# choyingw/SynergyNet

Measured on AMD Instinct MI355X. Metric: faces/sec (120x120, 68-lmk + 53215-vert), higher is better.
Workload: dtype f32 (fp16x2 split operands, fp32 accumulate)

## Files before the change

synergynet_amd/csrc/fused_block_lb.hip:

```cpp
#include "syn_internal.h"

#include <cstdio>
#include <cstdlib>

namespace syn {

typedef float f32x4 __attribute__((ext_vector_type(4)));
typedef float f32x2 __attribute__((ext_vector_type(2)));
typedef unsigned u32x4 __attribute__((ext_vector_type(4)));
typedef unsigned u32x2 __attribute__((ext_vector_type(2)));
typedef _Float16 f16x8 __attribute__((ext_vector_type(8)));
typedef _Float16 f16x2 __attribute__((ext_vector_type(2)));

namespace {
__device__ __forceinline__ void split2h(float x0, float x1, unsigned &a, unsigned &b) {
    a = __builtin_bit_cast(unsigned, __builtin_amdgcn_cvt_pkrtz(x0, x1));
    float r0, r1;
    asm("v_fma_mix_f32 %0, %1, -1.0, %2 op_sel_hi:[1,0,0]" : "=v"(r0) : "v"(a), "v"(x0));
    asm("v_fma_mix_f32 %0, %1, -1.0, %2 op_sel:[1,0,0] op_sel_hi:[1,0,0]" : "=v"(r1) : "v"(a), "v"(x1));
    b = __builtin_bit_cast(unsigned, __builtin_amdgcn_cvt_pkrtz(r0, r1));
}
__device__ __forceinline__ void split2v(float x0, float x1, u32x4 (&pc)[2], int d) {
    unsigned a, b;
    split2h(x0, x1, a, b);
// ... 34 lines not shown
__device__ __forceinline__ f32x2 pk_fma_clamp01(f32x2 a, f32x2 b, f32x2 c) {
    f32x2 r;
    asm("v_pk_fma_f32 %0, %1, %2, %3 clamp" : "=v"(r) : "v"(a), "v"(b), "v"(c));
    return r;
}
constexpr int kRowShr1 = 0x111, kRowShl1 = 0x101, kRowShr8 = 0x118, kRowShl8 = 0x108;
constexpr int kRowShr4 = 0x114, kRowShr5 = 0x115;
}

template <int CIN_, int HID_, int COUT_, bool RES_, int EPF_, int PPF_, int FPW_ = 2, bool S2_ = false, int NS_ = 2>
struct LbCfg {
    static constexpr int CIN = CIN_, HID = HID_, COUT = COUT_, FPW = FPW_;
    static constexpr int PPF = PPF_;
    static constexpr bool TLATE = false;
    static constexpr int EPF = EPF_;
    static constexpr bool RES = RES_;
    static constexpr bool S2 = S2_;
    static constexpr int NB = S2 ? 1 : 4;
    static constexpr int PIXO = NB * 16;
    static constexpr int KE = CIN / 32;
    static constexpr int NG = HID / 32;
    static constexpr int MT = COUT / 16;
    static constexpr int NS = NS_;
    static constexpr int NW = FPW * NS, NT = NW * 64;
    static constexpr int XF_DW = KE * 4 * 2 * 256;
    static constexpr int NSX = NS == 8 ? 4 : NS;
    static constexpr int KT = (MT + NSX - 1) / NSX;
    static constexpr int RED_DW = (NS == 2 ? 1 : NSX) * MT * NB * 256;
    static constexpr int TB_DW = 12 * 32;
    static constexpr int FACE_DW = XF_DW > RED_DW ? XF_DW : RED_DW;
    static constexpr int LDS_DW = FPW * FACE_DW + NW * TB_DW;
    static_assert(CIN % 32 == 0 && HID % 64 == 0 && COUT % 32 == 0, "k32 steps, two streams, two halves of the output tiles");
    static_assert(NS == 2 || (NS == 8 && FPW == 1 && (HID / 32) >= NS), "eight streams: the one-face-per-workgroup schedule of small batches (the four-stream form of round 4 is retired)");
    static_assert(EPF == 1 || EPF == KE, "expand prefetch depth");
    static_assert(!RES || (CIN == COUT && !S2), "residual only on same-width stride-1 blocks");
    static_assert((FPW == 4 || NS >= 4 ? 1 : 2) * LDS_DW * 4 <= 160 * 1024, "one 8-wave or two 4-wave workgroups per CU");
};

#define SYNL_FENCE() do { asm volatile("" ::: "memory"); __builtin_amdgcn_sched_barrier(0); } while (0)

#define SYNL_LAP(i) do { if (PROF) { tn = __builtin_amdgcn_s_memtime(); pt_[i] += tn - tk; tk = tn; } } while (0)

struct LbStageArgs {
    const float *X;
    const unsigned *Weh;
    const float *Tlb;
    const unsigned *Wlb;
    const float *p_shift;
    float *Y;
    float *part = nullptr;
    int gsl = 0;
};

template <class C, class CN, bool FIRST, bool PROF, int FACE_DW, bool STORE = true, bool PARTIAL = false, int RED_OFF = 0>
__device__ __forceinline__ void lb_stage(unsigned *smem, const LbStageArgs &sa, int B, unsigned long long (&pt_)[5], unsigned long long &tk) {
    unsigned long long tn = 0;
    const float *__restrict__ X = sa.X;
    const unsigned *__restrict__ Weh = sa.Weh, *__restrict__ Wlb = sa.Wlb;
    const float *__restrict__ Tlb = sa.Tlb, *__restrict__ p_shift = sa.p_shift;
    float *__restrict__ Y = sa.Y;
    constexpr int KE = C::KE, MT = C::MT, CIN = C::CIN, COUT = C::COUT, NB = C::NB;
    const int tid = threadIdx.x, lane = tid & 63;
    const int wave = __builtin_amdgcn_readfirstlane(tid >> 6);
    const int fl = wave / C::NS, st = wave % C::NS;
    const int f = blockIdx.x * C::FPW + fl;
    const bool real = f < B;
    const int fc = real ? f : B - 1;
    const int n = lane & 15, g = lane >> 4;
    const unsigned l4 = lane * 4, g4 = g * 4;
    unsigned *Xf = smem + fl * FACE_DW;
    constexpr int BPW = 4 / C::NS;
    auto pix_in = [&](int b, int nn) __attribute__((always_inline)) {
        return C::S2 ? 16 * (nn >> 2) + 8 * (b >> 1) + 2 * (nn & 3) + (b & 1) : 32 * (nn >> 3) + (nn & 7) + 8 * b;
    };

    if constexpr (FIRST && C::NS == 8) {
        constexpr int NIT = (KE * 4 + 7) / 8;
        f32x4 xv[NIT][2];
#pragma unroll
        for (int i = 0; i < NIT; ++i) {
            const int it = st + 8 * i, itc = it < KE * 4 ? it : 0;
            const float *src = X + ((size_t)fc * 64 + pix_in(itc & 3, n)) * CIN + 32 * (itc >> 2) + 8 * g;
            xv[i][0] = *(const f32x4 *)src;
            xv[i][1] = *(const f32x4 *)(src + 4);
        }
#pragma unroll
        for (int i = 0; i < NIT; ++i) {
            const int it = st + 8 * i;
            f32x4 a = xv[i][0], b = xv[i][1];
            if (!real) { a = (f32x4){0.f, 0.f, 0.f, 0.f}; b = a; }
            a *= 16.0f; b *= 16.0f;
            u32x4 pc[2];
            split2v(a[0], a[1], pc, 0);
            split2v(a[2], a[3], pc, 1);
            split2v(b[0], b[1], pc, 2);
            split2v(b[2], b[3], pc, 3);
            if (it < KE * 4) {
#pragma unroll
                for (int p = 0; p < 2; ++p) *(u32x4 *)&Xf[(it * 2 + p) * 256 + lane * 4] = pc[p];
            }
        }
    } else if (FIRST) {
        f32x4 xv[KE][BPW][2];
#pragma unroll
        for (int kc = 0; kc < KE; ++kc)
#pragma unroll
            for (int rr = 0; rr < BPW; ++rr) {
// ... 145 lines not shown
            for (int r = 0; r < NB; ++r) {
                split2v(O[r][0], O[r][1], Bd[r], th);
                if (hf) {
#pragma unroll
                    for (int p = 0; p < 2; ++p) asm volatile("" : "+v"(Bd[r][p]));
                }
            }
            SYNL_FENCE();
        }
        SYNL_LAP(2);
        const bool more = G + C::NS < gend;
#pragma unroll
        for (int i = 1; i < C::PPF; ++i)
            if (i < MT) fetch_p(i);
        if (more) {
            if (!C::TLATE) fetch_t(G + C::NS);
            if (C::EPF != KE) {
#pragma unroll
                for (int kc = 0; kc < C::EPF; ++kc) fetch_e(G + C::NS, kc);
            }
        }
        if constexpr (C::S2) {
            static_assert(!C::S2 || (C::PPF == 2 && MT % 2 == 0), "output tiles in pairs, two tiles fetched ahead");
#pragma unroll
            for (int mt = 0; mt < MT; mt += 2) {
                if (mt + 2 < MT) { fetch_p(mt + 2); fetch_p(mt + 3); }
                constexpr int PA[3] = {1, 0, 0}, PB[3] = {0, 1, 0};
#pragma unroll
                for (int j = 0; j < 3; ++j) {
                    acc[mt][0] = mfmal(Ap[mt % RING][PA[j]], Bd[0][PB[j]], acc[mt][0]);
                    acc[mt + 1][0] = mfmal(Ap[(mt + 1) % RING][PA[j]], Bd[0][PB[j]], acc[mt + 1][0]);
                }
                SYNL_FENCE();
            }
        } else {
#pragma unroll
            for (int mt = 0; mt < MT; ++mt) {
                if (mt + C::PPF < MT) fetch_p(mt + C::PPF);
                mac3x4(Ap[mt % RING], Bd[0], acc[mt][0], Ap[mt % RING], Bd[1], acc[mt][1], Ap[mt % RING], Bd[2], acc[mt][2], Ap[mt % RING], Bd[3], acc[mt][3]);
                SYNL_FENCE();
            }
        }
        if (more) {
            if (C::TLATE) fetch_t(G + C::NS);
            park_t();
        }
        SYNL_LAP(3);
    }

    float *Red = reinterpret_cast<float *>(Xf + RED_OFF);
    int le = lane;
    asm volatile("" : "+v"(le));
    const int ne = le & 15, ge = le >> 4, pixe = C::S2 ? ne : 32 * (ne >> 3) + (ne & 7);
    const __amdgpu_buffer_rsrc_t rs_x = __builtin_amdgcn_make_buffer_rsrc(const_cast<float *>(X), 0, 0x7fffffff, 0x00027000);
    constexpr int KT = C::KT, NSW = C::NSX;
    f32x4 rs[KT][NB], psh[KT];
#pragma unroll
    for (int i = 0; i < KT; ++i) {
        const int mtk = NSW * i + (st & (NSW - 1));
        const int nch = 16 * (mtk < MT ? mtk : MT - 1) + 4 * ge;
        psh[i] = *(const f32x4 *)&p_shift[nch];
#pragma unroll
        for (int r = 0; r < NB; ++r)
            if (C::RES && !PARTIAL) rs[i][r] = __builtin_bit_cast(f32x4, __builtin_amdgcn_raw_buffer_load_b128(rs_x, (unsigned)(((fc * 64 + pixe + 8 * r) * COUT + nch) * 4), 0, FIRST ? 0 : 1));
    }
    if (RED_OFF == 0) __syncthreads();
    constexpr bool HANDOFF = !__is_same(CN, void);
    f32x4 vout[KT][NB];
    if constexpr (C::NS == 2) {
#pragma unroll
    for (int mt = 0; mt < MT; ++mt) {
        if ((mt & 1) == st) continue;
#pragma unroll
        for (int r = 0; r < NB; ++r) *(f32x4 *)&Red[(((st * (MT / 2) + (mt >> 1)) * NB + r) * 64 + lane) * 4] = acc[mt][r];
    }
    __syncthreads();
#pragma unroll
    for (int mt = 0; mt < MT; ++mt) {
        if ((mt & 1) != st) continue;
        const int nch = 16 * mt + 4 * ge;
#pragma unroll
        for (int r = 0; r < NB; ++r) {
            const f32x4 o = *(const f32x4 *)&Red[((((1 - st) * (MT / 2) + (mt >> 1)) * NB + r) * 64 + lane) * 4];
            f32x4 v = st == 0 ? acc[mt][r] + o : o + acc[mt][r];
            if constexpr (PARTIAL) {
                if (real) *(f32x4 *)&sa.part[(((size_t)blockIdx.y * B + f) * C::PIXO + pixe + 8 * r) * COUT + nch] = v;
                continue;
            }
            v = v * inv_p + psh[mt >> 1];
            if (C::RES) v += rs[mt >> 1][r];
            if (STORE && real) *(f32x4 *)&Y[((size_t)f * C::PIXO + pixe + 8 * r) * COUT + nch] = v;
            if (HANDOFF) vout[mt >> 1][r] = v;
        }
    }
    } else {
        static_assert(!PARTIAL, "the four-stream schedule reduces inside the workgroup");
        if constexpr (C::NS == 8) {
            if (st >= 4) {
#pragma unroll
                for (int mt = 0; mt < MT; ++mt)
#pragma unroll
                    for (int r = 0; r < NB; ++r) *(f32x4 *)&Red[((((st - 4) * MT + mt) * NB + r) * 64 + lane) * 4] = acc[mt][r];
            }
            __syncthreads();
            if (st < 4) {
#pragma unroll
                for (int mt = 0; mt < MT; ++mt)
#pragma unroll
                    for (int r = 0; r < NB; ++r) acc[mt][r] += *(const f32x4 *)&Red[(((st * MT + mt) * NB + r) * 64 + lane) * 4];
            }
            __syncthreads();
        }
#pragma unroll
        for (int mt = 0; mt < MT; ++mt) {
            if (mt % NSW == st || st >= NSW) continue;
#pragma unroll
            for (int r = 0; r < NB; ++r) *(f32x4 *)&Red[(((st * MT + mt) * NB + r) * 64 + lane) * 4] = acc[mt][r];
        }
        __syncthreads();
#pragma unroll
        for (int mt = 0; mt < MT; ++mt) {
            if (mt % NSW != st) continue;
            const int nch = 16 * mt + 4 * ge;
#pragma unroll
            for (int r = 0; r < NB; ++r) {
                f32x4 v = st == 0 ? acc[mt][r] : *(const f32x4 *)&Red[(((0 * MT + mt) * NB + r) * 64 + lane) * 4];
#pragma unroll
                for (int so = 1; so < NSW; ++so) v += so == st ? acc[mt][r] : *(const f32x4 *)&Red[(((so * MT + mt) * NB + r) * 64 + lane) * 4];
                v = v * inv_p + psh[mt / NSW];
                if (C::RES) v += rs[mt / NSW][r];
                if (STORE && real) *(f32x4 *)&Y[((size_t)f * C::PIXO + pixe + 8 * r) * COUT + nch] = v;
                if (HANDOFF) vout[mt / NSW][r] = v;
            }
        }
    }
    if constexpr (HANDOFF) {
        static_assert(CN::CIN == COUT && !C::S2, "the next block of the chain takes this block's output (8x8)");
        if (RED_OFF == 0) __syncthreads();
#pragma unroll
        for (int mt = 0; mt < MT; ++mt) {
            if (mt % NSW != st) continue;
            const int kc = mt >> 1, lg = (2 * (mt & 1) + (ge >> 1)) * 16, dw = 2 * (ge & 1);
#pragma unroll
            for (int r = 0; r < 4; ++r) {
                const f32x4 v = real ? vout[mt / NSW][r] * 16.0f : (f32x4){0.f, 0.f, 0.f, 0.f};
                unsigned a0, b0, a1, b1;
                split2h(v[0], v[1], a0, b0);
                split2h(v[2], v[3], a1, b1);
                const int bn = CN::S2 ? 2 * (r & 1) + (ne & 1) : r;
                const int nn = CN::S2 ? 4 * ((r >> 1) + 2 * (ne >> 3)) + ((ne & 7) >> 1) : ne;
                *(u32x2 *)&Xf[((kc * 4 + bn) * 2 + 0) * 256 + (lg + nn) * 4 + dw] = (u32x2){a0, a1};
                *(u32x2 *)&Xf[((kc * 4 + bn) * 2 + 1) * 256 + (lg + nn) * 4 + dw] = (u32x2){b0, b1};
            }
        }
    }
    SYNL_LAP(4);
}

struct L7 {
    static constexpr int CIN = 32, HID = 192, COUT = 64, NG = 6, MT = 4, H = 15, HO = 8;
    static constexpr int FPW = 2, NW = 4, NT = 256;
    static constexpr int XF_DW = 16 * 2 * 256;
    static constexpr int TB_DW = 12 * 32;
    static constexpr int FACE_DW = XF_DW;
    static constexpr int LDS_DW = FPW * FACE_DW + NW * TB_DW;
};

template <class CN, bool PROF, int FACE_DW>
__device__ __forceinline__ void lb7_stage(unsigned *smem, const LbStageArgs &sa, int B, unsigned long long (&pt_)[5], unsigned long long &tk) {
    unsigned long long tn = 0;
    const float *__restrict__ X = sa.X;
    const float *__restrict__ Tlb = sa.Tlb, *__restrict__ p_shift = sa.p_shift;
    float *__restrict__ Y = sa.Y;
    constexpr int MT = L7::MT, CIN = L7::CIN, COUT = L7::COUT;
    const int tid = threadIdx.x, lane = tid & 63;
    const int wave = __builtin_amdgcn_readfirstlane(tid >> 6);
    const int fl = wave >> 1, st = wave & 1;
    const int f = blockIdx.x * L7::FPW + fl;
    const bool real = f < B;
    const int fc = real ? f : B - 1;
    const int n = lane & 15, g = lane >> 4;
    const unsigned l4 = lane * 4, g4 = g * 4;
    unsigned *Xf = smem + fl * FACE_DW;

#pragma unroll
    for (int hb = 0; hb < 2; ++hb) {
        f32x4 xv[4][2];
        bool ok[4];
#pragma unroll
        for (int b = 0; b < 4; ++b) {
            const int y = 2 * (2 * b + (n >> 3)) + st, x = 2 * (n & 7) + hb;
            ok[b] = real && y < L7::H && x < L7::H;
            const float *src = X + ((size_t)fc * (L7::H * L7::H) + (ok[b] ? y * L7::H + x : 0)) * CIN + 8 * g;
            xv[b][0] = *(const f32x4 *)src;
            xv[b][1] = *(const f32x4 *)(src + 4);
        }
#pragma unroll
        for (int b = 0; b < 4; ++b) {
            f32x4 a = xv[b][0], c = xv[b][1];
            if (!ok[b]) { a = (f32x4){0.f, 0.f, 0.f, 0.f}; c = a; }
            a *= 16.0f; c *= 16.0f;
            u32x4 pc[2];
            split2v(a[0], a[1], pc, 0);
            split2v(a[2], a[3], pc, 1);
            split2v(c[0], c[1], pc, 2);
            split2v(c[2], c[3], pc, 3);
#pragma unroll
            for (int p = 0; p < 2; ++p) *(u32x4 *)&Xf[((((2 * st + hb) * 4 + b) * 2) + p) * 256 + lane * 4] = pc[p];
        }
    }
    const float mL = (n & 7) != 0 ? 1.f : 0.f;
    f32x4 acc[MT][2];
#pragma unroll
    for (int mt = 0; mt < MT; ++mt)
#pragma unroll
        for (int k = 0; k < 2; ++k) acc[mt][k] = (f32x4){0.f, 0.f, 0.f, 0.f};

    float *Tb = reinterpret_cast<float *>(smem + L7::FPW * FACE_DW + wave * L7::TB_DW);
    const __amdgpu_buffer_rsrc_t rs_e = __builtin_amdgcn_make_buffer_rsrc(const_cast<unsigned *>(sa.Weh), 0, 0x7fffffff, 0x00027000);
    const __amdgpu_buffer_rsrc_t rs_p = __builtin_amdgcn_make_buffer_rsrc(const_cast<unsigned *>(sa.Wlb), 0, 0x7fffffff, 0x00027000);
    const __amdgpu_buffer_rsrc_t rs_t = __builtin_amdgcn_make_buffer_rsrc(const_cast<float *>(Tlb), 0, 0x7fffffff, 0x00027000);
// ... 78 lines not shown
            };
            f32x2 up2, up3;
            if (st == 1) {
                up2 = dpp2<kRowShl8>(relu(D[t][2][2], c6e));
                up3 = dpp2<kRowShl8>(relu(D[t][3][2], cJ));
            } else {
                up2 = (f32x2){0.f, 0.f}; up3 = up2;
            }
#pragma unroll
            for (int k = 0; k < 2; ++k) {
                const f32x2 E0 = relu(D[t][0][k], c6e), E1 = relu(D[t][1][k], cJ);
                const f32x2 E2 = relu(D[t][2][k], k == 1 ? cR0 : c6e), E3 = relu(D[t][3][k], k == 1 ? cR1 : cJ);
                const f32x2 U2 = dpp2<kRowShr8>(E2) + up2, U3 = dpp2<kRowShr8>(E3) + up3;
                f32x2 O = dsh;
                O += dpp2<kRowShr1>(U3) * w[0];
                O += U2 * w[1];
                O += U3 * w[2];
                asm volatile("" : "+v"(O));
                O += dpp2<kRowShr1>(E1) * w[3];
                O += E0 * w[4];
                O += E1 * w[5];
                asm volatile("" : "+v"(O));
                O += dpp2<kRowShr1>(E3) * w[6];
                O += E2 * w[7];
                O = pk_fma_clamp01(E3, w[8], O);
                split2v(O[0], O[1], Bd[k], th);
                if (k == 0) { up2 = dpp2<kRowShl8>(E2); up3 = dpp2<kRowShl8>(E3); }
            }
            SYNL_FENCE();
        }
        SYNL_LAP(2);
        const bool more = G + 1 < L7::NG;
        fetch_p(1);
        if (more) { fetch_t(G + 1); fetch_e(G + 1); }
#pragma unroll
        for (int mt = 0; mt < MT; ++mt) {
            if (mt + 2 < MT) fetch_p(mt + 2);
            constexpr int PA[3] = {1, 0, 0}, PB[3] = {0, 1, 0};
#pragma unroll
            for (int j = 0; j < 3; ++j) {
                acc[mt][0] = mfmal(Ap[mt % 3][PA[j]], Bd[0][PB[j]], acc[mt][0]);
                acc[mt][1] = mfmal(Ap[mt % 3][PA[j]], Bd[1][PB[j]], acc[mt][1]);
            }
            SYNL_FENCE();
        }
        if (more) park_t();
        SYNL_LAP(3);
    }

    int le = lane;
    asm volatile("" : "+v"(le));
    const int ne = le & 15, ge = le >> 4, ox = ne & 7;
    constexpr bool HANDOFF = !__is_same(CN, void);
    if constexpr (HANDOFF) __syncthreads();
#pragma unroll
    for (int mt = 0; mt < MT; ++mt) {
        const int nch = 16 * mt + 4 * ge;
        const f32x4 psh = *(const f32x4 *)&p_shift[nch];
#pragma unroll
        for (int k = 0; k < 2; ++k) {
            const int oy = 4 * st + 2 * k + (ne >> 3);
            const f32x4 v = acc[mt][k] * inv_p + psh;
            if (real) *(f32x4 *)&Y[((size_t)f * 64 + oy * 8 + ox) * COUT + nch] = v;
            if constexpr (HANDOFF) {
                static_assert(CN::CIN == COUT && !CN::S2, "features.8 takes this block's output");
                const int kc = mt >> 1, lg = (2 * (mt & 1) + (ge >> 1)) * 16, dw = 2 * (ge & 1);
                const int r = 2 * k + (ne >> 3), nn = 8 * st + ox;
                const f32x4 vs = real ? v * 16.0f : (f32x4){0.f, 0.f, 0.f, 0.f};
                unsigned a0, b0, a1, b1;
                split2h(vs[0], vs[1], a0, b0);
                split2h(vs[2], vs[3], a1, b1);
                *(u32x2 *)&Xf[((kc * 4 + r) * 2 + 0) * 256 + (lg + nn) * 4 + dw] = (u32x2){a0, a1};
                *(u32x2 *)&Xf[((kc * 4 + r) * 2 + 1) * 256 + (lg + nn) * 4 + dw] = (u32x2){b0, b1};
            }
        }
    }
    SYNL_LAP(4);
}

template <class CN, int FACE_DW>
__device__ __forceinline__ void lb7_stage8(unsigned *smem, const LbStageArgs &sa, int B) {
    const float *__restrict__ X = sa.X;
    const float *__restrict__ Tlb = sa.Tlb, *__restrict__ p_shift = sa.p_shift;
    float *__restrict__ Y = sa.Y;
    constexpr int MT = L7::MT, CIN = L7::CIN, COUT = L7::COUT;
    const int tid = threadIdx.x, lane = tid & 63;
    const int wave = __builtin_amdgcn_readfirstlane(tid >> 6);
    const int q = wave & 3, hs = wave >> 2;
    const int f = blockIdx.x;
    const bool real = f < B;
    const int fc = real ? f : B - 1;
    const int n = lane & 15, g = lane >> 4;
    const unsigned l4 = lane * 4, g4 = g * 4;
    unsigned *Xf = smem;

    {
        const int c = wave & 3, py = c >> 1, px = c & 1, b0 = 2 * (wave >> 2);
        f32x4 xv[2][2];
        bool ok[2];
#pragma unroll
        for (int bb = 0; bb < 2; ++bb) {
            const int b = b0 + bb;
            const int y = 2 * (2 * b + (n >> 3)) + py, x = 2 * (n & 7) + px;
            ok[bb] = real && y < L7::H && x < L7::H;
            const float *src = X + ((size_t)fc * (L7::H * L7::H) + (ok[bb] ? y * L7::H + x : 0)) * CIN + 8 * g;
            xv[bb][0] = *(const f32x4 *)src;
            xv[bb][1] = *(const f32x4 *)(src + 4);
        }
#pragma unroll
        for (int bb = 0; bb < 2; ++bb) {
            f32x4 a = xv[bb][0], d = xv[bb][1];
            if (!ok[bb]) { a = (f32x4){0.f, 0.f, 0.f, 0.f}; d = a; }
            a *= 16.0f; d *= 16.0f;
            u32x4 pc[2];
            split2v(a[0], a[1], pc, 0);
            split2v(a[2], a[3], pc, 1);
            split2v(d[0], d[1], pc, 2);
            split2v(d[2], d[3], pc, 3);
#pragma unroll
            for (int p = 0; p < 2; ++p) *(u32x4 *)&Xf[(((c * 4 + b0 + bb) * 2) + p) * 256 + lane * 4] = pc[p];
        }
    }
    const float mL = (n & 7) != 0 ? 1.f : 0.f;
    f32x4 acc[MT];
#pragma unroll
    for (int mt = 0; mt < MT; ++mt) acc[mt] = (f32x4){0.f, 0.f, 0.f, 0.f};

    float *Tb = reinterpret_cast<float *>(smem + FACE_DW + wave * L7::TB_DW);
    const __amdgpu_buffer_rsrc_t rs_e = __builtin_amdgcn_make_buffer_rsrc(const_cast<unsigned *>(sa.Weh), 0, 0x7fffffff, 0x00027000);
    const __amdgpu_buffer_rsrc_t rs_p = __builtin_amdgcn_make_buffer_rsrc(const_cast<unsigned *>(sa.Wlb), 0, 0x7fffffff, 0x00027000);
    const __amdgpu_buffer_rsrc_t rs_t = __builtin_amdgcn_make_buffer_rsrc(const_cast<float *>(Tlb), 0, 0x7fffffff, 0x00027000);
    const unsigned l16 = lane * 16;
    f32x4 tv[2];
// ... 76 lines not shown
                up2 = dpp2<kRowShl8>(relu(Dh[t][0], c6e));
                up3 = dpp2<kRowShl8>(relu(Dh[t][1], cJ));
            } else {
                up2 = (f32x2){0.f, 0.f}; up3 = up2;
            }
            const f32x2 E0 = relu(D[t][0], c6e), E1 = relu(D[t][1], cJ);
            const f32x2 E2 = relu(D[t][2], cR0), E3 = relu(D[t][3], cR1);
            const f32x2 U2 = dpp2<kRowShr8>(E2) + up2, U3 = dpp2<kRowShr8>(E3) + up3;
            f32x2 O = dsh;
            O += dpp2<kRowShr1>(U3) * w[0];
            O += U2 * w[1];
            O += U3 * w[2];
            asm volatile("" : "+v"(O));
            O += dpp2<kRowShr1>(E1) * w[3];
            O += E0 * w[4];
            O += E1 * w[5];
            asm volatile("" : "+v"(O));
            O += dpp2<kRowShr1>(E3) * w[6];
            O += E2 * w[7];
            O = pk_fma_clamp01(E3, w[8], O);
            split2v(O[0], O[1], Bd, th);
            SYNL_FENCE();
        }
        const bool more = G + 2 < L7::NG;
        fetch_p(1);
        if (more) { fetch_t(G + 2); fetch_e(G + 2); }
#pragma unroll
        for (int mt = 0; mt < MT; ++mt) {
            if (mt + 2 < MT) fetch_p(mt + 2);
            constexpr int PA[3] = {1, 0, 0}, PB[3] = {0, 1, 0};
#pragma unroll
            for (int j = 0; j < 3; ++j) acc[mt] = mfmal(Ap[mt % 3][PA[j]], Bd[PB[j]], acc[mt]);
            SYNL_FENCE();
        }
        if (more) park_t();
    }

    float *Ex = reinterpret_cast<float *>(Xf);
    int le = lane;
    asm volatile("" : "+v"(le));
    const int ne = le & 15, ge = le >> 4, ox = ne & 7, oy = 2 * q + (ne >> 3);
    __syncthreads();
    if (hs == 1) {
#pragma unroll
        for (int mt = 0; mt < MT; ++mt) *(f32x4 *)&Ex[((q * MT + mt) * 64 + lane) * 4] = acc[mt];
    }
    __syncthreads();
    f32x4 v[MT];
    if (hs == 0) {
#pragma unroll
        for (int mt = 0; mt < MT; ++mt) {
            const int nch = 16 * mt + 4 * ge;
            v[mt] = (acc[mt] + *(const f32x4 *)&Ex[((q * MT + mt) * 64 + lane) * 4]) * inv_p + *(const f32x4 *)&p_shift[nch];
            if (real) *(f32x4 *)&Y[((size_t)f * 64 + oy * 8 + ox) * COUT + nch] = v[mt];
        }
    }
    static_assert(CN::CIN == COUT && !CN::S2, "features.8 takes this block's output");
    __syncthreads();
    if (hs == 0) {
#pragma unroll
        for (int mt = 0; mt < MT; ++mt) {
            const int kc = mt >> 1, lg = (2 * (mt & 1) + (ge >> 1)) * 16, dw = 2 * (ge & 1);
            const int r = oy & 3, nn = 8 * (oy >> 2) + ox;
            const f32x4 vs = real ? v[mt] * 16.0f : (f32x4){0.f, 0.f, 0.f, 0.f};
            unsigned a0, b0, a1, b1;
            split2h(vs[0], vs[1], a0, b0);
            split2h(vs[2], vs[3], a1, b1);
            *(u32x2 *)&Xf[((kc * 4 + r) * 2 + 0) * 256 + (lg + nn) * 4 + dw] = (u32x2){a0, a1};
            *(u32x2 *)&Xf[((kc * 4 + r) * 2 + 1) * 256 + (lg + nn) * 4 + dw] = (u32x2){b0, b1};
        }
    }
}

template <bool PROF = false>
__global__ __launch_bounds__(L7::NT) __attribute__((amdgpu_waves_per_eu(2, 2)))
void fused_block_lb7_kernel(LbStageArgs sa, int B, unsigned long long *prof = nullptr) {
    unsigned long long pt_[5] = {0, 0, 0, 0, 0}, tk = PROF ? __builtin_amdgcn_s_memtime() : 0ull;
    __shared__ __attribute__((aligned(16))) unsigned smem[L7::LDS_DW];
    lb7_stage<void, PROF, L7::FACE_DW>(smem, sa, B, pt_, tk);
    if (PROF && (threadIdx.x & 63) == 0) {
        for (int i = 0; i < 5; ++i) atomicAdd(&prof[i], pt_[i]);
        atomicAdd(&prof[7], 1ull);
    }
}

template <class C, bool PROF = false, bool PARTIAL = false>
__global__ __launch_bounds__(C::NT) __attribute__((amdgpu_waves_per_eu(2, 2)))
void fused_block_lb_kernel(LbStageArgs sa, int B, unsigned long long *prof = nullptr) {
    unsigned long long pt_[5] = {0, 0, 0, 0, 0}, tk = PROF ? __builtin_amdgcn_s_memtime() : 0ull;
    __shared__ __attribute__((aligned(16))) unsigned smem[C::LDS_DW];
    lb_stage<C, void, true, PROF, C::FACE_DW, true, PARTIAL>(smem, sa, B, pt_, tk);
    if (PROF && (threadIdx.x & 63) == 0) {
        for (int i = 0; i < 5; ++i) atomicAdd(&prof[i], pt_[i]);
        atomicAdd(&prof[7], 1ull);
    }
}

using L8 = LbCfg<      64, 384,  64, true,  2, 3>;
using L11 = LbCfg<     64, 384,  96, false, 2, 3>;
using L12 = LbCfg<     96, 576,  96, true,  1, 3>;
using L14 = LbCfg<     96, 576, 160, false, 1, 2, 2, true>;

struct LbChainArgs { LbStageArgs s[8]; };
constexpr int kChainFaceDw = L7::FACE_DW;
static_assert(L8::FACE_DW <= kChainFaceDw && L11::FACE_DW <= kChainFaceDw && L12::FACE_DW <= kChainFaceDw && L14::FACE_DW <= kChainFaceDw,
              "every stage reuses the fragment buffers of the first");
constexpr int kChainLdsDw = L8::FPW * kChainFaceDw + L8::NW * L8::TB_DW;
static_assert(2 * kChainLdsDw * 4 <= 160 * 1024, "two workgroups per CU");

template <int NG, int KE, int MT>
__device__ __forceinline__ void lb_touch_stage(const LbStageArgs &sa, unsigned gi, unsigned nth, unsigned &sink) {
    l2_touch(sa.Weh, NG * KE * 4096u, gi, nth, sink);
    l2_touch(sa.Wlb, NG * MT * 2048u, gi, nth, sink);
    l2_touch(sa.Tlb, NG * 12u * 32u * 4u, gi, nth, sink);
}
template <bool WITH7, bool WITH14>
__global__ __launch_bounds__(L8::NT) __attribute__((amdgpu_waves_per_eu(2, 2)))
void fused_chain_lb_kernel(LbChainArgs ca, int B) {
    unsigned long long pt_[5] = {0, 0, 0, 0, 0}, tk = 0;
    __shared__ __attribute__((aligned(16))) unsigned smem[kChainLdsDw];
    unsigned sink = 0;
    const unsigned gi = (blockIdx.x >> 3) * (unsigned)L8::NT + threadIdx.x, nth = ((gridDim.x + 7) >> 3) * (unsigned)L8::NT;
    if (WITH7) lb_touch_stage<L7::NG, 1, L7::MT>(ca.s[0], gi, nth, sink);
    lb_touch_stage<L8::NG, L8::KE, L8::MT>(ca.s[1], gi, nth, sink);
    lb_touch_stage<L8::NG, L8::KE, L8::MT>(ca.s[2], gi, nth, sink);
    lb_touch_stage<L8::NG, L8::KE, L8::MT>(ca.s[3], gi, nth, sink);
    lb_touch_stage<L11::NG, L11::KE, L11::MT>(ca.s[4], gi, nth, sink);
    lb_touch_stage<L12::NG, L12::KE, L12::MT>(ca.s[5], gi, nth, sink);
    lb_touch_stage<L12::NG, L12::KE, L12::MT>(ca.s[6], gi, nth, sink);
    if (WITH14) lb_touch_stage<L14::NG, L14::KE, L14::MT>(ca.s[7], gi, nth, sink);
    if constexpr (WITH7) {
        lb7_stage<L8, false, kChainFaceDw>(smem, ca.s[0], B, pt_, tk);
        lb_stage<L8, L8, false, false, kChainFaceDw>(smem, ca.s[1], B, pt_, tk);
    } else
        lb_stage<L8, L8, true, false, kChainFaceDw>(smem, ca.s[1], B, pt_, tk);
    lb_stage<L8, L8, false, false, kChainFaceDw>(smem, ca.s[2], B, pt_, tk);
    lb_stage<L8, L11, false, false, kChainFaceDw>(smem, ca.s[3], B, pt_, tk);
    lb_stage<L11, L12, false, false, kChainFaceDw>(smem, ca.s[4], B, pt_, tk);
    lb_stage<L12, L12, false, false, kChainFaceDw>(smem, ca.s[5], B, pt_, tk);
    if constexpr (WITH14) {
        lb_stage<L12, L14, false, false, kChainFaceDw, false>(smem, ca.s[6], B, pt_, tk);
        lb_stage<L14, void, false, false, kChainFaceDw>(smem, ca.s[7], B, pt_, tk);
    } else
        lb_stage<L12, void, false, false, kChainFaceDw>(smem, ca.s[6], B, pt_, tk);
    l2_touch_done(sink);
}

constexpr int cmax4(int a, int b, int c, int d) { return (a > b ? a : b) > (c > d ? c : d) ? (a > b ? a : b) : (c > d ? c : d); }

using L8e = LbCfg<     64, 384,  64, true,  2, 3, 1, false, 8>;
using L11e = LbCfg<    64, 384,  96, false, 2, 3, 1, false, 8>;
using L12e = LbCfg<    96, 576,  96, true,  1, 3, 1, false, 8>;
using L14e = LbCfg<    96, 576, 160, false, 1, 2, 1, true, 8>;
constexpr int kChainXfDwE = cmax4(L7::XF_DW, L8e::XF_DW, L12e::XF_DW, L14e::XF_DW);
constexpr int kChainRedDwE = cmax4(L8e::RED_DW, L11e::RED_DW, L12e::RED_DW, L14e::RED_DW);
constexpr int kRedOffE = kChainXfDwE;
constexpr int kFaceDwE = kChainXfDwE + kChainRedDwE;
constexpr int kLdsDwE = kFaceDwE + L8e::NW * L8e::TB_DW;
static_assert(kLdsDwE * 4 <= 160 * 1024, "one workgroup per CU");
template <bool WITH7 = false>
__global__ __launch_bounds__(L8e::NT) __attribute__((amdgpu_waves_per_eu(2, 2)))
void fused_chain_lb_small8_kernel(LbChainArgs ca, int B) {
    unsigned long long pt_[5] = {0, 0, 0, 0, 0}, tk = 0;
    __shared__ __attribute__((aligned(16))) unsigned smem[kLdsDwE];
    if constexpr (WITH7) {
        lb7_stage8<L8e, kFaceDwE>(smem, ca.s[0], B);
        lb_stage<L8e, L8e, false, false, kFaceDwE, true, false, kRedOffE>(smem, ca.s[1], B, pt_, tk);
    } else
    lb_stage<L8e, L8e, true, false, kFaceDwE, true, false, kRedOffE>(smem, ca.s[1], B, pt_, tk);
    lb_stage<L8e, L8e, false, false, kFaceDwE, true, false, kRedOffE>(smem, ca.s[2], B, pt_, tk);
    lb_stage<L8e, L11e, false, false, kFaceDwE, true, false, kRedOffE>(smem, ca.s[3], B, pt_, tk);
    lb_stage<L11e, L12e, false, false, kFaceDwE, true, false, kRedOffE>(smem, ca.s[4], B, pt_, tk);
    lb_stage<L12e, L12e, false, false, kFaceDwE, true, false, kRedOffE>(smem, ca.s[5], B, pt_, tk);
    lb_stage<L12e, L14e, false, false, kFaceDwE, false, false, kRedOffE>(smem, ca.s[6], B, pt_, tk);
    lb_stage<L14e, void, false, false, kFaceDwE, true, false, kRedOffE>(smem, ca.s[7], B, pt_, tk);
}

template <class C>
__global__ __launch_bounds__(256) void lb_reduce_kernel(const float *__restrict__ part, int S, const float *__restrict__ Tlb,
                                                        const float *__restrict__ p_shift, const float *__restrict__ X,
                                                        float *__restrict__ Y, int B) {
    constexpr int C4 = C::COUT / 4;
    const long idx = (long)blockIdx.x * 256 + threadIdx.x, total = (long)B * C::PIXO * C4;
    if (idx >= total) return;
    const int c4 = (int)(idx % C4);
    const float inv_p = Tlb[11 * 32 + 1];
    f32x4 a = *(const f32x4 *)&part[(size_t)idx * 4];
    for (int sl = 1; sl < S; ++sl) a += *(const f32x4 *)&part[((size_t)sl * total + idx) * 4];
    f32x4 v = a * inv_p + *(const f32x4 *)&p_shift[4 * c4];
    if (C::RES) v += *(const f32x4 *)&X[(size_t)idx * 4];
    *(f32x4 *)&Y[(size_t)idx * 4] = v;
}

template <class C>
static bool launch_lb_sliced(const FusedBlockArgs &a, int B, hipStream_t s) {
    if (!a.scratch || a.prof) return false;
    const int wg = (B + C::FPW - 1) / C::FPW;
    int S = 0;
    for (int d = 2; d <= C::NG / 2; ++d)
        if (C::NG % d == 0) { S = d; if (wg * d >= 256) break; }
    if (S < 2 || (size_t)S * B * C::PIXO * C::COUT > a.scratch_floats) return false;
    LbStageArgs sa{a.X, a.Alb_e, a.Tlb, a.Alb_p, a.p_shift, a.Y};
    sa.part = a.scratch; sa.gsl = C::NG / S;
    fused_block_lb_kernel<C, false, true><<<dim3(wg, S), C::NT, 0, s>>>(sa, B);
    const long total = (long)B * C::PIXO * (C::COUT / 4);
    lb_reduce_kernel<C><<<(int)((total + 255) / 256), 256, 0, s>>>(a.scratch, S, a.Tlb, a.p_shift, a.X, a.Y, B);
    return true;
}

template <class C>
static void launch_lb(const FusedBlockArgs &a, int B, hipStream_t s) {
    const int grid = (B + C::FPW - 1) / C::FPW;
    const LbStageArgs sa{a.X, a.Alb_e, a.Tlb, a.Alb_p, a.p_shift, a.Y};
    if (a.prof) fused_block_lb_kernel<C, true><<<grid, C::NT, 0, s>>>(sa, B, a.prof);
    else fused_block_lb_kernel<C><<<grid, C::NT, 0, s>>>(sa, B);
}

constexpr int kChainMin = 384;
constexpr int kSmallChainMax = 256;
static bool small_f7() {
    static const bool on = test_knob("small_f7", 1) != 0;
    return on;
}
int lb_chain_mode(int B, bool small) {
    static const int chain = (int)test_knob("lb_chain", 3);
    if (chain <= 0) return 0;
    if (B < kChainMin) return (small && B <= kSmallChainMax) ? (small_f7() ? 3 : 2) : 0;
    return chain > 3 ? 3 : chain;
}
bool launch_fused_chain_lb(const FusedBlockArgs *a, int first, int n_blocks, int B, hipStream_t s) {
    const int last = first + n_blocks - 1;
    if ((first != 7 && first != 8) || (last != 13 && last != 14) || (first == 7 && last != 14)) return false;
    LbChainArgs ca;
    for (int i = 0; i < n_blocks; ++i) {
        if (!a[i].Alb_e || !a[i].Alb_p || !a[i].Tlb || a[i].prof) return false;
        ca.s[first - 7 + i] = LbStageArgs{a[i].X, a[i].Alb_e, a[i].Tlb, a[i].Alb_p, a[i].p_shift, a[i].Y};
    }
    if (first == 8) ca.s[0] = ca.s[1];
    if (last == 13) ca.s[7] = ca.s[6];
    if (B < kChainMin) {
        if (last != 14 || (first == 7 && !small_f7())) return false;
        if (first == 7) { fused_chain_lb_small8_kernel<true><<<B, L8e::NT, 0, s>>>(ca, B); return true; }
        fused_chain_lb_small8_kernel<false><<<B, L8e::NT, 0, s>>>(ca, B);
        return true;
    }
    const int grid = (B + L8::FPW - 1) / L8::FPW;
    if (first == 7) fused_chain_lb_kernel<true, true><<<grid, L8::NT, 0, s>>>(ca, B);
    else if (last == 14) fused_chain_lb_kernel<false, true><<<grid, L8::NT, 0, s>>>(ca, B);
    else fused_chain_lb_kernel<false, false><<<grid, L8::NT, 0, s>>>(ca, B);
    return true;
}

constexpr int kLbMinBatch = 768;

bool launch_fused_block_lb(int feature, const FusedBlockArgs &a, int B, hipStream_t s) {
    if (!a.Alb_e || !a.Alb_p || !a.Tlb) return false;
    if (B < kLbMinBatch) {
        constexpr int sl_min = 32, narrow_max = 192;
        if (B < sl_min || feature < 8 || (feature < 12 && B > narrow_max)) return false;
        switch (feature) {
            case 8: case 9: case 10: return launch_lb_sliced<L8>(a, B, s);
            case 11: return launch_lb_sliced<L11>(a, B, s);
            case 12: case 13: return launch_lb_sliced<L12>(a, B, s);
            case 14: return launch_lb_sliced<L14>(a, B, s);
            default: return false;
        }
    }
    switch (feature) {
        case 7: {
            const LbStageArgs sa{a.X, a.Alb_e, a.Tlb, a.Alb_p, a.p_shift, a.Y};
            const int grid = (B + L7::FPW - 1) / L7::FPW;
            if (a.prof) fused_block_lb7_kernel<true><<<grid, L7::NT, 0, s>>>(sa, B, a.prof);
            else fused_block_lb7_kernel<false><<<grid, L7::NT, 0, s>>>(sa, B);
            return true;
        }
        case 8: case 9: case 10: launch_lb<L8>(a, B, s); return true;
        case 11: launch_lb<L11>(a, B, s); return true;
        case 12: case 13: launch_lb<L12>(a, B, s); return true;
        case 14: launch_lb<L14>(a, B, s); return true;
        default: return false;
    }
}

}
```

Before: 1.007 million.

## Park residual tiles in LDS across fused chain stages instead of global round-trips

Each stage of the fused MobileNet-style chain now writes the tiles of its output that the next stage needs as a residual into a spare region of the face's LDS buffer. The next stage reads those tiles from LDS instead of reloading them from global memory. Where a stage's output is only consumed inside the kernel, the global store is dropped. This removes global load and store traffic for residuals at the cost of extra LDS use and layout constraints, which are checked by static asserts. It is gated by a knob that is on by default.

```diff
diff --git a/synergynet_amd/csrc/fused_block_lb.hip b/synergynet_amd/csrc/fused_block_lb.hip
--- a/synergynet_amd/csrc/fused_block_lb.hip
+++ b/synergynet_amd/csrc/fused_block_lb.hip
@@ -110,7 +110,15 @@
     int gsl = 0;
 };
 
-template <class C, class CN, bool FIRST, bool PROF, int FACE_DW, bool STORE = true, bool PARTIAL = false, int RED_OFF = 0>
+template <class C, int RED_OFF, int FACE_DW>
+struct LbPark {
+    static constexpr int OFF = RED_OFF ? C::XF_DW : C::FACE_DW;
+    static constexpr int TILE_DW = C::NSX * C::NB * 256;
+    static constexpr int ROOM = ((RED_OFF ? RED_OFF : FACE_DW) - OFF) / TILE_DW;
+    static constexpr int KP = ROOM < C::KT ? (ROOM < 0 ? 0 : ROOM) : C::KT;
+    static constexpr int END = OFF + KP * TILE_DW;
+};
+template <class C, class CN, bool FIRST, bool PROF, int FACE_DW, bool STORE = true, bool PARTIAL = false, int RED_OFF = 0, int RL = 0>
 __device__ __forceinline__ void lb_stage(unsigned *smem, const LbStageArgs &sa, int B, unsigned long long (&pt_)[5], unsigned long long &tk) {
     unsigned long long tn = 0;
     const float *__restrict__ X = sa.X;
@@ -362,6 +370,13 @@
     int le = lane;
     asm volatile("" : "+v"(le));
     const int ne = le & 15, ge = le >> 4, pixe = C::S2 ? ne : 32 * (ne >> 3) + (ne & 7);
+    constexpr bool RIN = (RL & 1) != 0, ROUT = (RL & 2) != 0;
+    static_assert(!RIN || (C::RES && !FIRST && !PARTIAL), "a parked residual needs the stage in front of it in the same kernel");
+    using PC = LbPark<C, RED_OFF, FACE_DW>;
+    static_assert(!RIN || (PC::KP >= 1 && PC::OFF >= C::XF_DW && (RED_OFF ? PC::END <= RED_OFF : (PC::OFF >= C::RED_DW && PC::END <= FACE_DW))),
+                  "the park lies clear of this stage's fragments and exchange buffer, inside the face buffer");
+    constexpr int KPI = RIN ? PC::KP : 0;
+    const float *Pk = reinterpret_cast<const float *>(Xf + PC::OFF) + (st & (C::NSX - 1)) * (KPI * NB * 256);
     const __amdgpu_buffer_rsrc_t rs_x = __builtin_amdgcn_make_buffer_rsrc(const_cast<float *>(X), 0, 0x7fffffff, 0x00027000);
     constexpr int KT = C::KT, NSW = C::NSX;
     f32x4 rs[KT][NB], psh[KT];
@@ -372,10 +387,20 @@
         psh[i] = *(const f32x4 *)&p_shift[nch];
 #pragma unroll
         for (int r = 0; r < NB; ++r)
-            if (C::RES && !PARTIAL) rs[i][r] = __builtin_bit_cast(f32x4, __builtin_amdgcn_raw_buffer_load_b128(rs_x, (unsigned)(((fc * 64 + pixe + 8 * r) * COUT + nch) * 4), 0, FIRST ? 0 : 1));
+            if (C::RES && !PARTIAL && i >= KPI) rs[i][r] = __builtin_bit_cast(f32x4, __builtin_amdgcn_raw_buffer_load_b128(rs_x, (unsigned)(((fc * 64 + pixe + 8 * r) * COUT + nch) * 4), 0, FIRST ? 0 : 1));
     }
     if (RED_OFF == 0) __syncthreads();
     constexpr bool HANDOFF = !__is_same(CN, void);
+    static_assert(!ROUT || HANDOFF, "parking is for the next stage");
+    float *Pko = nullptr;
+    constexpr int KPO = [] { if constexpr (ROUT) return LbPark<CN, RED_OFF, FACE_DW>::KP; else return 0; }();
+    if constexpr (ROUT) {
+        using PN = LbPark<CN, RED_OFF, FACE_DW>;
+        static_assert(CN::RES && CN::NS == C::NS && CN::MT == MT && CN::NB == NB && KPO >= 1, "the next stage's residual is this output, tile for tile");
+        static_assert(PN::OFF >= C::XF_DW && PN::OFF >= CN::XF_DW && (RED_OFF ? PN::END <= RED_OFF : (PN::OFF >= C::RED_DW && PN::END <= FACE_DW)),
+                      "clear of what this stage still reads and of the fragments it hands over");
+        Pko = reinterpret_cast<float *>(Xf + PN::OFF) + (st & (C::NSX - 1)) * (KPO * NB * 256);
+    }
     f32x4 vout[KT][NB];
     if constexpr (C::NS == 2) {
 #pragma unroll
@@ -398,8 +423,9 @@
                 continue;
             }
             v = v * inv_p + psh[mt >> 1];
-            if (C::RES) v += rs[mt >> 1][r];
-            if (STORE && real) *(f32x4 *)&Y[((size_t)f * C::PIXO + pixe + 8 * r) * COUT + nch] = v;
+            if (C::RES) v += (mt >> 1) < KPI ? *(const f32x4 *)&Pk[(((mt >> 1) * NB + r) * 64 + lane) * 4] : rs[mt >> 1][r];
+            if (STORE && (mt >> 1) >= KPO && real) *(f32x4 *)&Y[((size_t)f * C::PIXO + pixe + 8 * r) * COUT + nch] = v;
+            if ((mt >> 1) < KPO) *(f32x4 *)&Pko[(((mt >> 1) * NB + r) * 64 + lane) * 4] = v;
             if (HANDOFF) vout[mt >> 1][r] = v;
         }
     }
@@ -438,8 +464,9 @@
 #pragma unroll
                 for (int so = 1; so < NSW; ++so) v += so == st ? acc[mt][r] : *(const f32x4 *)&Red[(((so * MT + mt) * NB + r) * 64 + lane) * 4];
                 v = v * inv_p + psh[mt / NSW];
-                if (C::RES) v += rs[mt / NSW][r];
-                if (STORE && real) *(f32x4 *)&Y[((size_t)f * C::PIXO + pixe + 8 * r) * COUT + nch] = v;
+                if (C::RES) v += (mt / NSW) < KPI ? *(const f32x4 *)&Pk[(((mt / NSW) * NB + r) * 64 + lane) * 4] : rs[mt / NSW][r];
+                if (STORE && (mt / NSW) >= KPO && real) *(f32x4 *)&Y[((size_t)f * C::PIXO + pixe + 8 * r) * COUT + nch] = v;
+                if ((mt / NSW) < KPO) *(f32x4 *)&Pko[(((mt / NSW) * NB + r) * 64 + lane) * 4] = v;
                 if (HANDOFF) vout[mt / NSW][r] = v;
             }
         }
@@ -476,7 +503,7 @@
     static constexpr int LDS_DW = FPW * FACE_DW + NW * TB_DW;
 };
 
-template <class CN, bool PROF, int FACE_DW>
+template <class CN, bool PROF, int FACE_DW, bool STORE = true, bool PARK = false>
 __device__ __forceinline__ void lb7_stage(unsigned *smem, const LbStageArgs &sa, int B, unsigned long long (&pt_)[5], unsigned long long &tk) {
     unsigned long long tn = 0;
     const float *__restrict__ X = sa.X;
@@ -661,6 +688,7 @@
     asm volatile("" : "+v"(le));
     const int ne = le & 15, ge = le >> 4, ox = ne & 7;
     constexpr bool HANDOFF = !__is_same(CN, void);
+    static_assert(HANDOFF || (STORE && !PARK), "a block on its own stores its output");
     if constexpr (HANDOFF) __syncthreads();
 #pragma unroll
     for (int mt = 0; mt < MT; ++mt) {
@@ -670,11 +698,16 @@
         for (int k = 0; k < 2; ++k) {
             const int oy = 4 * st + 2 * k + (ne >> 3);
             const f32x4 v = acc[mt][k] * inv_p + psh;
-            if (real) *(f32x4 *)&Y[((size_t)f * 64 + oy * 8 + ox) * COUT + nch] = v;
+            if (STORE && real) *(f32x4 *)&Y[((size_t)f * 64 + oy * 8 + ox) * COUT + nch] = v;
             if constexpr (HANDOFF) {
                 static_assert(CN::CIN == COUT && !CN::S2, "features.8 takes this block's output");
                 const int kc = mt >> 1, lg = (2 * (mt & 1) + (ge >> 1)) * 16, dw = 2 * (ge & 1);
                 const int r = 2 * k + (ne >> 3), nn = 8 * st + ox;
+                if constexpr (PARK) {
+                    using PN = LbPark<CN, 0, FACE_DW>;
+                    static_assert(CN::NS == 2 && CN::MT == MT && PN::KP == CN::KT && PN::OFF >= CN::XF_DW && PN::END <= FACE_DW, "features.8's park, clear of the fragments written below");
+                    *(f32x4 *)&reinterpret_cast<float *>(Xf + PN::OFF)[((((mt & 1) * CN::KT + (mt >> 1)) * 4 + r) * 64 + 16 * ge + nn) * 4] = v;
+                }
                 const f32x4 vs = real ? v * 16.0f : (f32x4){0.f, 0.f, 0.f, 0.f};
                 unsigned a0, b0, a1, b1;
                 split2h(vs[0], vs[1], a0, b0);
@@ -687,7 +720,7 @@
     SYNL_LAP(4);
 }
 
-template <class CN, int FACE_DW>
+template <class CN, int FACE_DW, int RED_OFF, bool PARK = false>
 __device__ __forceinline__ void lb7_stage8(unsigned *smem, const LbStageArgs &sa, int B) {
     const float *__restrict__ X = sa.X;
     const float *__restrict__ Tlb = sa.Tlb, *__restrict__ p_shift = sa.p_shift;
@@ -870,7 +903,7 @@
         for (int mt = 0; mt < MT; ++mt) {
             const int nch = 16 * mt + 4 * ge;
             v[mt] = (acc[mt] + *(const f32x4 *)&Ex[((q * MT + mt) * 64 + lane) * 4]) * inv_p + *(const f32x4 *)&p_shift[nch];
-            if (real) *(f32x4 *)&Y[((size_t)f * 64 + oy * 8 + ox) * COUT + nch] = v[mt];
+            if (!PARK && real) *(f32x4 *)&Y[((size_t)f * 64 + oy * 8 + ox) * COUT + nch] = v[mt];
         }
     }
     static_assert(CN::CIN == COUT && !CN::S2, "features.8 takes this block's output");
@@ -880,6 +913,12 @@
         for (int mt = 0; mt < MT; ++mt) {
             const int kc = mt >> 1, lg = (2 * (mt & 1) + (ge >> 1)) * 16, dw = 2 * (ge & 1);
             const int r = oy & 3, nn = 8 * (oy >> 2) + ox;
+            if constexpr (PARK) {
+                using PN = LbPark<CN, RED_OFF, FACE_DW>;
+                static_assert(CN::NS == 8 && CN::KT == 1 && PN::KP == 1 && CN::MT == MT && PN::OFF >= CN::XF_DW && PN::OFF >= MT * 4 * 256 && PN::END <= RED_OFF,
+                              "features.8's park, clear of the fragments written below and of the exchange buffer read above");
+                *(f32x4 *)&reinterpret_cast<float *>(Xf + PN::OFF)[((mt * 4 + r) * 64 + 16 * ge + nn) * 4] = v[mt];
+            }
             const f32x4 vs = real ? v[mt] * 16.0f : (f32x4){0.f, 0.f, 0.f, 0.f};
             unsigned a0, b0, a1, b1;
             split2h(vs[0], vs[1], a0, b0);
@@ -932,7 +971,7 @@
     l2_touch(sa.Wlb, NG * MT * 2048u, gi, nth, sink);
     l2_touch(sa.Tlb, NG * 12u * 32u * 4u, gi, nth, sink);
 }
-template <bool WITH7, bool WITH14>
+template <bool WITH7, bool WITH14, int RL>
 __global__ __launch_bounds__(L8::NT) __attribute__((amdgpu_waves_per_eu(2, 2)))
 void fused_chain_lb_kernel(LbChainArgs ca, int B) {
     unsigned long long pt_[5] = {0, 0, 0, 0, 0}, tk = 0;
@@ -947,20 +986,21 @@
     lb_touch_stage<L12::NG, L12::KE, L12::MT>(ca.s[5], gi, nth, sink);
     lb_touch_stage<L12::NG, L12::KE, L12::MT>(ca.s[6], gi, nth, sink);
     if (WITH14) lb_touch_stage<L14::NG, L14::KE, L14::MT>(ca.s[7], gi, nth, sink);
+    constexpr int IN = RL ? 1 : 0, OUT = RL ? 2 : 0, IN12 = RL == 2 ? 1 : 0, OUT12 = RL == 2 ? 2 : 0;
     if constexpr (WITH7) {
-        lb7_stage<L8, false, kChainFaceDw>(smem, ca.s[0], B, pt_, tk);
-        lb_stage<L8, L8, false, false, kChainFaceDw>(smem, ca.s[1], B, pt_, tk);
+        lb7_stage<L8, false, kChainFaceDw, !RL, RL != 0>(smem, ca.s[0], B, pt_, tk);
+        lb_stage<L8, L8, false, false, kChainFaceDw, !RL, false, 0, IN | OUT>(smem, ca.s[1], B, pt_, tk);
     } else
-        lb_stage<L8, L8, true, false, kChainFaceDw>(smem, ca.s[1], B, pt_, tk);
-    lb_stage<L8, L8, false, false, kChainFaceDw>(smem, ca.s[2], B, pt_, tk);
-    lb_stage<L8, L11, false, false, kChainFaceDw>(smem, ca.s[3], B, pt_, tk);
-    lb_stage<L11, L12, false, false, kChainFaceDw>(smem, ca.s[4], B, pt_, tk);
-    lb_stage<L12, L12, false, false, kChainFaceDw>(smem, ca.s[5], B, pt_, tk);
+        lb_stage<L8, L8, true, false, kChainFaceDw, !RL, false, 0, OUT>(smem, ca.s[1], B, pt_, tk);
+    lb_stage<L8, L8, false, false, kChainFaceDw, !RL, false, 0, IN | OUT>(smem, ca.s[2], B, pt_, tk);
+    lb_stage<L8, L11, false, false, kChainFaceDw, false, false, 0, IN>(smem, ca.s[3], B, pt_, tk);
+    lb_stage<L11, L12, false, false, kChainFaceDw, true, false, 0, OUT12>(smem, ca.s[4], B, pt_, tk);
+    lb_stage<L12, L12, false, false, kChainFaceDw, true, false, 0, IN12 | OUT12>(smem, ca.s[5], B, pt_, tk);
     if constexpr (WITH14) {
-        lb_stage<L12, L14, false, false, kChainFaceDw, false>(smem, ca.s[6], B, pt_, tk);
+        lb_stage<L12, L14, false, false, kChainFaceDw, false, false, 0, IN12>(smem, ca.s[6], B, pt_, tk);
         lb_stage<L14, void, false, false, kChainFaceDw>(smem, ca.s[7], B, pt_, tk);
     } else
-        lb_stage<L12, void, false, false, kChainFaceDw>(smem, ca.s[6], B, pt_, tk);
+        lb_stage<L12, void, false, false, kChainFaceDw, true, false, 0, IN12>(smem, ca.s[6], B, pt_, tk);
     l2_touch_done(sink);
 }
 
@@ -976,18 +1016,19 @@
 constexpr int kFaceDwE = kChainXfDwE + kChainRedDwE;
 constexpr int kLdsDwE = kFaceDwE + L8e::NW * L8e::TB_DW;
 static_assert(kLdsDwE * 4 <= 160 * 1024, "one workgroup per CU");
-template <bool WITH7 = false>
+template <bool WITH7, bool RL>
 __global__ __launch_bounds__(L8e::NT) __attribute__((amdgpu_waves_per_eu(2, 2)))
 void fused_chain_lb_small8_kernel(LbChainArgs ca, int B) {
     unsigned long long pt_[5] = {0, 0, 0, 0, 0}, tk = 0;
     __shared__ __attribute__((aligned(16))) unsigned smem[kLdsDwE];
+    constexpr int IN = RL ? 1 : 0, OUT = RL ? 2 : 0;
     if constexpr (WITH7) {
-        lb7_stage8<L8e, kFaceDwE>(smem, ca.s[0], B);
-        lb_stage<L8e, L8e, false, false, kFaceDwE, true, false, kRedOffE>(smem, ca.s[1], B, pt_, tk);
+        lb7_stage8<L8e, kFaceDwE, kRedOffE, RL>(smem, ca.s[0], B);
+        lb_stage<L8e, L8e, false, false, kFaceDwE, !RL, false, kRedOffE, IN | OUT>(smem, ca.s[1], B, pt_, tk);
     } else
-    lb_stage<L8e, L8e, true, false, kFaceDwE, true, false, kRedOffE>(smem, ca.s[1], B, pt_, tk);
-    lb_stage<L8e, L8e, false, false, kFaceDwE, true, false, kRedOffE>(smem, ca.s[2], B, pt_, tk);
-    lb_stage<L8e, L11e, false, false, kFaceDwE, true, false, kRedOffE>(smem, ca.s[3], B, pt_, tk);
+    lb_stage<L8e, L8e, true, false, kFaceDwE, !RL, false, kRedOffE, OUT>(smem, ca.s[1], B, pt_, tk);
+    lb_stage<L8e, L8e, false, false, kFaceDwE, !RL, false, kRedOffE, IN | OUT>(smem, ca.s[2], B, pt_, tk);
+    lb_stage<L8e, L11e, false, false, kFaceDwE, false, false, kRedOffE, IN>(smem, ca.s[3], B, pt_, tk);
     lb_stage<L11e, L12e, false, false, kFaceDwE, true, false, kRedOffE>(smem, ca.s[4], B, pt_, tk);
     lb_stage<L12e, L12e, false, false, kFaceDwE, true, false, kRedOffE>(smem, ca.s[5], B, pt_, tk);
     lb_stage<L12e, L14e, false, false, kFaceDwE, false, false, kRedOffE>(smem, ca.s[6], B, pt_, tk);
@@ -1056,16 +1097,30 @@
     }
     if (first == 8) ca.s[0] = ca.s[1];
     if (last == 13) ca.s[7] = ca.s[6];
+    static const int res_lds = (int)test_knob("lb_res_lds", 1);
     if (B < kChainMin) {
         if (last != 14 || (first == 7 && !small_f7())) return false;
-        if (first == 7) { fused_chain_lb_small8_kernel<true><<<B, L8e::NT, 0, s>>>(ca, B); return true; }
-        fused_chain_lb_small8_kernel<false><<<B, L8e::NT, 0, s>>>(ca, B);
+        if (first == 7) {
+            if (res_lds) fused_chain_lb_small8_kernel<true, true><<<B, L8e::NT, 0, s>>>(ca, B);
+            else fused_chain_lb_small8_kernel<true, false><<<B, L8e::NT, 0, s>>>(ca, B);
+        } else {
+            if (res_lds) fused_chain_lb_small8_kernel<false, true><<<B, L8e::NT, 0, s>>>(ca, B);
+            else fused_chain_lb_small8_kernel<false, false><<<B, L8e::NT, 0, s>>>(ca, B);
+        }
         return true;
     }
     const int grid = (B + L8::FPW - 1) / L8::FPW;
-    if (first == 7) fused_chain_lb_kernel<true, true><<<grid, L8::NT, 0, s>>>(ca, B);
-    else if (last == 14) fused_chain_lb_kernel<false, true><<<grid, L8::NT, 0, s>>>(ca, B);
-    else fused_chain_lb_kernel<false, false><<<grid, L8::NT, 0, s>>>(ca, B);
+    if (first == 7) {
+        if (res_lds >= 2) fused_chain_lb_kernel<true, true, 2><<<grid, L8::NT, 0, s>>>(ca, B);
+        else if (res_lds) fused_chain_lb_kernel<true, true, 1><<<grid, L8::NT, 0, s>>>(ca, B);
+        else fused_chain_lb_kernel<true, true, 0><<<grid, L8::NT, 0, s>>>(ca, B);
+    } else if (last == 14) {
+        if (res_lds) fused_chain_lb_kernel<false, true, 1><<<grid, L8::NT, 0, s>>>(ca, B);
+        else fused_chain_lb_kernel<false, true, 0><<<grid, L8::NT, 0, s>>>(ca, B);
+    } else {
+        if (res_lds) fused_chain_lb_kernel<false, false, 1><<<grid, L8::NT, 0, s>>>(ca, B);
+        else fused_chain_lb_kernel<false, false, 0><<<grid, L8::NT, 0, s>>>(ca, B);
+    }
     return true;
 }
 
```

After: 1.006 million. Within noise of the previous version (-0.1%).
